# Tongji-MIC-Lab/TDVC

Measured on AMD Instinct MI355X. Metric: 1080p P-frames/sec (encode + reconstruct, lambda=2048 config), higher is better.
Workload: dtype f16; 1 GPU; 1x 1920x1080 (padded 1088x1920) 7-frame synthetic GOP (seed 1234), batch 1, P-frames coded in GOP order; gop=7, batch=1, parallelism=gop-sharded x1, weights=closed-form filler (no checkpoint ships)

## Files before the change

### include/tdvc_hip.h

```cpp
#ifndef TDVC_HIP_H
#define TDVC_HIP_H

#include <stdint.h>

#ifdef __cplusplus
extern "C" {
#endif

#define TDVC_OK 0
#define TDVC_EINVAL (-1)
#define TDVC_ENOSUP (-2)

typedef struct {
  void* p;
  int32_t N, H, W, C;
  int64_t sn;
  int32_t sp;
  int32_t dtype;
} tdvc_fmap;

enum { TDVC_F16 = 0, TDVC_F32 = 1 };
enum { TDVC_ACT_NONE = 0, TDVC_ACT_RELU = 1, TDVC_ACT_LRELU = 2, TDVC_ACT_CLAMP01 = 3, TDVC_ACT_SIGMOID = 4 };
enum { TDVC_GDN_NONE = 0, TDVC_GDN_FWD = 1, TDVC_GDN_INV = 2 };
enum { TDVC_OUT_NHWC = 0,
// ... 18 lines not shown
  int32_t act; float slope;
  int32_t round_before_act;
  tdvc_fmap res;
  tdvc_fmap res2;
  int32_t out_mode;
  int32_t s2d;
  int32_t bcast_T;
  float bcast_slope;
  float* chan_sum;
} tdvc_conv_desc;

int tdvc_abi_version(void);
const char* tdvc_last_error(void);
int tdvc_prepare_device(void);
const char* tdvc_last_conv_kernel(void);


int tdvc_conv_plan(int cin, int kh, int kw, int stride);
int64_t tdvc_conv_packed_bytes(int cout, int cin, int ntaps, int ck);
int tdvc_pack_conv_weights(const float* w_oihw, int cout, int cin_real, int cin, int kh, int kw,
                           int ntaps, const int8_t* tap_dy, const int8_t* tap_dx, int ck, uint16_t* dst);
int tdvc_conv2d(const tdvc_conv_desc* d, void* stream);
int tdvc_conv_chan_sum_rows(const tdvc_conv_desc* d);
const char* tdvc_conv_select(const tdvc_conv_desc* d);
int tdvc_conv2d_f32(const tdvc_conv_desc* d, void* stream);

typedef struct {
  tdvc_fmap x, y;
  const void* w;
  const float* bias;
// ... 222 lines not shown
```

### tdvc_amd/_lib.py

```python
from __future__ import annotations

import ctypes as C
import os

_HERE = os.path.dirname(os.path.abspath(__file__))
LIB_PATH = os.path.join(_HERE, "libtdvc_hip.so")

MAX_TAPS = 49
F16, F32 = 0, 1
ACT_NONE, ACT_RELU, ACT_LRELU, ACT_CLAMP01, ACT_SIGMOID = 0, 1, 2, 3, 4
GDN_NONE, GDN_FWD, GDN_INV = 0, 1, 2
OUT_NHWC, OUT_SHUFFLE2, OUT_NCHW_F32 = 0, 1, 2


class FMapDesc(C.Structure):
    _fields_ = [("p", C.c_void_p), ("N", C.c_int32), ("H", C.c_int32), ("W", C.c_int32), ("C", C.c_int32),
                ("sn", C.c_int64), ("sp", C.c_int32), ("dtype", C.c_int32)]


class ConvDesc(C.Structure):
    _fields_ = [("x", FMapDesc), ("y", FMapDesc), ("w", C.c_void_p), ("bias", C.c_void_p),
                ("cout", C.c_int32), ("ntaps", C.c_int32),
                ("tap_dy", C.c_int8 * MAX_TAPS), ("tap_dx", C.c_int8 * MAX_TAPS),
                ("kh", C.c_int32), ("kw", C.c_int32), ("stride", C.c_int32), ("pad", C.c_int32),
# ... 19 lines not shown
                ("nworkers", C.c_int32), ("cow", C.c_int32), ("ciw", C.c_int32), ("ntaps", C.c_int32), ("cout", C.c_int32), ("cin", C.c_int32),
                ("wblocks", C.c_int32), ("nblocks", C.c_int32)]


_P = C.c_void_p
_FM = C.POINTER(FMapDesc)
_i, _f, _i64 = C.c_int, C.c_float, C.c_int64

SIGNATURES = {
    "tdvc_abi_version": (_i, []),
    "tdvc_conv_chan_sum_rows": (_i, [C.POINTER(ConvDesc)]),
    "tdvc_conv_select": (C.c_char_p, [C.POINTER(ConvDesc)]),
    "tdvc_last_error": (C.c_char_p, []),
    "tdvc_last_conv_kernel": (C.c_char_p, []),
    "tdvc_prepare_device": (_i, []),
    "tdvc_conv_plan": (_i, [_i, _i, _i, _i]),
    "tdvc_conv_packed_bytes": (_i64, [_i, _i, _i, _i]),
    "tdvc_pack_conv_weights": (_i, [_P, _i, _i, _i, _i, _i, _i, _P, _P, _i, _P]),
    "tdvc_conv2d": (_i, [C.POINTER(ConvDesc), _P]),
    "tdvc_conv2d_f32": (_i, [C.POINTER(ConvDesc), _P]),
    "tdvc_pack_conv_weights_indexed": (_i, [_P] * 7 + [_i] * 4 + [_P, _P]),
    "tdvc_pack_conv_weights_indexed_f32": (_i, [_P] * 7 + [_i] * 4 + [_P, _P]),
    "tdvc_pack_job_blocks": (_i64, [_i, _i, _i, _i]),
    "tdvc_pack_conv_weights_batch": (_i, [_P, _P, _i, _i, _P]),
    "tdvc_act_backward": (_i, [_FM, _FM, _FM, _i, _f, _FM, _P]),
    "tdvc_pixel_unshuffle": (_i, [_FM, _FM, _P]),
    "tdvc_bias_grad_work_floats": (_i64, [_i, _i]),
    "tdvc_bias_grad": (_i, [_FM, _i, _P, _f, _P, _P, _i64, _P]),
    "tdvc_copy_cast": (_i, [_FM, _FM, _P]),
    "tdvc_clamp01_backward": (_i, [_FM, _FM, _P]),
# ... 109 lines not shown
```

### tdvc_amd/csrc/common.h

```cpp
#pragma once
#include <hip/hip_runtime.h>
#include <stdint.h>
#include <stdio.h>
#include <string.h>

#include "../../include/tdvc_hip.h"

typedef _Float16 half_t;
typedef _Float16 half8 __attribute__((ext_vector_type(8)));
typedef _Float16 half4 __attribute__((ext_vector_type(4)));
typedef _Float16 half2v __attribute__((ext_vector_type(2)));
typedef float f32x16 __attribute__((ext_vector_type(16)));
typedef float f32x4 __attribute__((ext_vector_type(4)));

void tdvc_set_error(const char* fmt, ...);
int tdvc_scratch_pages(const void** zeros, void** dump);

#define TDVC_CHECK(cond, ...)            \
  do {                                   \
    if (!(cond)) {                       \
      tdvc_set_error(__VA_ARGS__);       \
      return TDVC_EINVAL;                \
    }                                    \
  } while (0)

static inline int tdvc_launch_status(const char* what) {
  hipError_t e = hipGetLastError();
  if (e != hipSuccess) {
    tdvc_set_error("%s: launch failed: %s", what, hipGetErrorString(e));
    return (int)e;
  }
  return TDVC_OK;
}

static inline bool aligned16(const void* p) { return (((uintptr_t)p) & 15) == 0; }
struct TdvcPerDeviceFlag {
  bool done[64] = {};
  bool& flag() {
    int dev = 0;
    if (hipGetDevice(&dev) != hipSuccess || dev < 0 || dev >= 64) dev = 0;
    return done[dev];
// ... 46 lines not shown
```

### tdvc_amd/csrc/conv_c8.hip

```cpp
#include "conv_common.h"

using convk::ConvParams;

namespace {

constexpr int NW_C8 = 4, NTHR_C8 = 256;
constexpr int EW_C8 = 32 * 144;
constexpr int LDS_C8 = 256 + NW_C8 * EW_C8;

__global__ __launch_bounds__(NTHR_C8, 4) void conv_c8_kernel(const ConvParams p, int tiles_x, int total_tiles) {
  extern __shared__ __attribute__((aligned(16))) unsigned char smem[];
  float* bias_s = reinterpret_cast<float*>(smem);
  const int tid = threadIdx.x, lane = tid & 63;
  const int wave = __builtin_amdgcn_readfirstlane(tid >> 6);
  const int hh = lane >> 5, r = lane & 31;
  if (tid < 64) bias_s[tid] = p.bias[tid];
  unsigned char* ew = smem + 256 + wave * EW_C8;

  half8 wa[2][5];
#pragma unroll
  for (int mt = 0; mt < 2; ++mt)
#pragma unroll
    for (int s = 0; s < 5; ++s) wa[mt][s] = *reinterpret_cast<const half8*>(p.w + (((long)mt * 5 + s) * 64 + lane) * 8);

  int tdy[5], tdx[5];
// ... 70 lines not shown
    }
  }
}

}

bool conv_c8_eligible(const tdvc_conv_desc* d, const ConvParams& p, int Ho, int Wo) {
  return convk::taps_dense(d, 3, 3, 1) && d->ck == 8 && d->stride == 1 && d->cout == 64 && d->x.C == 8 && !d->s2d && !d->square_input &&
         (long)Ho * Wo >= convk::LARGE_MAP_PIXELS &&
         convk::conv_is_lean(p) && !p.res.p && !p.res2.p && p.y.C >= 64 && (long)d->x.N * Ho * ((Wo + 31) / 32) < (1L << 30);
}

int launch_conv_c8(const ConvParams& p, int N, hipStream_t st) {
  ConvParams q = p;
  q.slope = convk::conv_simple_slope(p);
  const int tiles_x = (p.Wo + 31) / 32;
  const long total = (long)N * p.Ho * tiles_x;
  int grid = (int)((total + NW_C8 - 1) / NW_C8);
  if (grid > 256 * 4) grid = 256 * 4;
  hipLaunchKernelGGL(conv_c8_kernel, dim3(grid), dim3(NTHR_C8), LDS_C8, st, q, tiles_x, (int)total);
  return tdvc_launch_status("tdvc_conv2d(c8)");
}
```

### tdvc_amd/csrc/conv_common.h

```cpp
#pragma once
#include "common.h"

namespace convk {

struct ConvParams {
  const half_t* x; long x_sn; int x_sp; int H, W, Cin;
  const half_t* w; const float* bias;
  FMap y; int Ho, Wo; int cout;
  FMap aux; FMap res; FMap res2;
  int ntaps, kh, kw, pad;
  int in_stride;
  int nchunks, steps;
  int square, gdn, act; float slope; int round16, out_mode;
  int tiles_x;
  int simple;
  int s2d, Corig;
  int reverse;
  int bcast_T; float bcast_slope;
  float* csum;
  int8_t tap_dy[TDVC_MAX_TAPS], tap_dx[TDVC_MAX_TAPS];
};

enum ConvSwitch { SW_NONE = -1, SW_V2, SW_V3, SW_V5, SW_V7, SW_V9, SW_V10, SW_V11, SW_ROW, SW_C8, SW_N16, SW_GDN128, SW_COUNT };
int conv_on(int id);
long conv_v9_work_limit();

constexpr long LARGE_MAP_PIXELS = 8192;

inline bool taps_dense(const tdvc_conv_desc* d, int kh, int kw, int pad) {
  if (d->ntaps != kh * kw || d->kh != kh || d->kw != kw || d->pad != pad) return false;
  for (int t = 0; t < d->ntaps; ++t)
    if (d->tap_dy[t] != t / kw || d->tap_dx[t] != t % kw) return false;
  return true;
}

// ... 450 lines not shown
```

### tdvc_amd/csrc/conv_pair.hip

```cpp
#include <type_traits>

#include "conv_common.h"

namespace {

constexpr int BI = 2;
constexpr int TRING = 2 * BI;
constexpr int SRING = 2 * BI;
constexpr int T_LAG = 1 + BI;
constexpr int ID_LAG = 2 + BI;
template <int NCB> struct PairGeoBase;
template <> struct PairGeoBase<2> { static constexpr int PIECES = 5, XRING = 16, PF = 8, HD = 4; };
template <> struct PairGeoBase<4> { static constexpr int PIECES = 9, XRING = 10, PF = 4, HD = 2; };
template <int NCB> struct PairGeo : PairGeoBase<NCB> {
  using G = PairGeoBase<NCB>;
  static constexpr int PW = 16 * NCB - 2;
  static constexpr int NPX = PW + 4;
  static constexpr int ROWB = G::PIECES * 1024;
  static constexpr int TROWB = ROWB;
  static constexpr int SROW = 16 * NCB * 128;
  static constexpr int X0 = 0, T0 = G::XRING * ROWB, S0 = T0 + TRING * TROWB;
  static constexpr int LDS = S0 + SRING * SROW;
  static_assert(NPX * 128 <= ROWB, "ring row holds the strip's input pixels");
  static_assert(G::PF - G::XRING < -(BI - 1) - ID_LAG, "input ring: a DMA would land on a row whose identity a conv2 wave BI - 1 steps behind has not read (needs PF + 2 BI + 2 <= XRING)");
// ... 16 lines not shown
#define PAIR_MID_G 1
#endif

struct PairParams {
  const half_t* x; long x_sn; int x_sp;
  half_t* y; long y_sn; int y_sp;
  const half_t* res2; long r2_sn; int r2_sp;
  const half_t* w;
  const float* bias;
  const half_t* zeros;
  half_t* dump;
  int N, H, W;
  int strips, segs, seg_rows, jobs;
  float slope1, slope2;
  int experiment;
};

__device__ __forceinline__ int swz(int q) { return (int)((0x62654210u >> (4 * ((q >> 1) & 7))) & 7u); }

__device__ __forceinline__ void glds16(const half_t* gsrc, unsigned lds_dst) {
  unsigned keep;
  asm volatile("s_mov_b32 %0, m0\n\ts_mov_b32 m0, %2\n\ts_nop 0\n\tglobal_load_lds_dwordx4 %1, off\n\ts_mov_b32 m0, %0"
               : "=&s"(keep) : "v"(gsrc), "s"(lds_dst) : "memory");
}
__device__ __forceinline__ void pair_barrier(bool skip = false) {
  asm volatile("s_waitcnt lgkmcnt(0)" ::: "memory");
  if (!skip) __builtin_amdgcn_s_barrier();
  asm volatile("" ::: "memory");
}
template <int A>
// ... 3 lines not shown
    return __builtin_elementwise_max(v, z);
  } else if constexpr (A == 2) {
    return __builtin_elementwise_max(v, v * sl);
  } else {
    return v;
  }
}

template <int XRING> __device__ __forceinline__ int pair_slot(int kk) {
  if constexpr ((XRING & (XRING - 1)) == 0) return kk & (XRING - 1);
  else return __builtin_amdgcn_readfirstlane(kk) % XRING;
}

template <int NCB, int A1, int A2, bool ADDX, bool RES2, bool STAMP = false>
__global__ __launch_bounds__(NTHR, 1) void conv_pair_kernel(const PairParams p, long long* stamps = nullptr, int stamp_cap = 0) {
  using G = PairGeo<NCB>;
  constexpr int PW = G::PW, ROWB = G::ROWB, TROWB = G::TROWB, SROW = G::SROW, XRING = G::XRING, PF = G::PF, X0 = G::X0, T0 = G::T0, S0 = G::S0;
  constexpr int NF = 6 * NCB;
  constexpr int NIT = NCB / 2;
  long long st_busy = 0, st_vm = 0, st_bar = 0, st_n = 0;
  extern __shared__ __attribute__((aligned(1024))) unsigned char smem[];
  const unsigned lds0 = static_cast<unsigned>(reinterpret_cast<uintptr_t>(smem));
  const int tid = threadIdx.x, lane = tid & 63;
  const int wave = __builtin_amdgcn_readfirstlane(tid >> 6);
  const int grp = wave >> 2, wq = wave & 3;
  const int r16 = lane & 15, kb = lane >> 4;

  half8 wf[18];
#pragma unroll
  for (int f = 0; f < 18; ++f) wf[f] = *reinterpret_cast<const half8*>(p.w + ((((long)(grp * 4 + wq) * 18 + f) * 64 + lane) * 8));
// ... 359 lines not shown
  const int PWsel = 16 * ncb - 2;
  p.strips = (p.W + PWsel - 1) / PWsel;
  const long base = (long)p.N * p.strips;
  int best = 1;
  double best_eff = 0.;
  for (int sg = 1; sg <= 64 && (p.H + sg - 1) / sg >= 16; ++sg) {
    const int sr = (p.H + sg - 1) / sg, nseg = (p.H + sr - 1) / sr;
    const long jobs = base * nseg;
    const double eff = (double)jobs / (double)(((jobs + 255) / 256) * 256) * sr / (sr + 5.0);
    if (eff > best_eff + 1e-9) { best_eff = eff; best = sg; }
  }
  p.seg_rows = (p.H + best - 1) / best;
  p.segs = (p.H + p.seg_rows - 1) / p.seg_rows;
  p.jobs = (int)(base * p.segs);
  const int grid = p.jobs < 256 ? p.jobs : 256;
  auto go = [&](auto kern, int lds) -> int {
    hipError_t err = hipFuncSetAttribute(reinterpret_cast<const void*>(kern), hipFuncAttributeMaxDynamicSharedMemorySize, lds);
    if (err != hipSuccess) { tdvc_set_error("tdvc_conv_pair: hipFuncSetAttribute failed: %s", hipGetErrorString(err)); return (int)err; }
    hipLaunchKernelGGL(kern, dim3(grid), dim3(NTHR), lds, reinterpret_cast<hipStream_t>(stream), p, g_pair_stamps, g_pair_stamp_cap);
    return 0;
  };
  const bool resblock = d->act1 == TDVC_ACT_RELU && d->act2 == TDVC_ACT_NONE;
  const int sel = (resblock ? 4 : 0) + (d->add_input ? 2 : 0) + (d->res2.p ? 1 : 0);
  auto launch = [&](auto ncbc) -> int {
    constexpr int NCB = decltype(ncbc)::value;
    constexpr int lds = PairGeo<NCB>::LDS;
    switch (sel) {
      case 0: return go(&conv_pair_kernel<NCB, 2, 2, false, false>, lds);
      case 1: return go(&conv_pair_kernel<NCB, 2, 2, false, true>, lds);
      case 2: return go(&conv_pair_kernel<NCB, 2, 2, true, false>, lds);
// ... 12 lines not shown
```

### tdvc_amd/csrc/conv_row.hip

```cpp
#include <type_traits>

#include "conv_common.h"

using convk::ConvParams;

namespace {

enum { GEO_C128 = 0, GEO_C64 = 1, GEO_C128W = 2, GEO_S2D64 = 3 };
template <int GID> struct RowGeo;
template <> struct RowGeo<GEO_C128> { static constexpr int NKC = 4, KH = 3, KW = 3, SW = 32, NCG = 8, PIECES = 9, XRING = 8, PF = 6, HD = 4, DMA_POS = 1, CORIG = 128; static constexpr bool S2D = false; };
template <> struct RowGeo<GEO_C64> { static constexpr int NKC = 2, KH = 3, KW = 3, SW = 64, NCG = 4, PIECES = 9, XRING = 8, PF = 6, HD = 4, DMA_POS = 2, CORIG = 64; static constexpr bool S2D = false; };
template <> struct RowGeo<GEO_C128W> { static constexpr int NKC = 4, KH = 3, KW = 3, SW = 64, NCG = 4, PIECES = 17, XRING = 6, PF = 4, HD = 2, DMA_POS = 2, CORIG = 128; static constexpr bool S2D = false; };
template <> struct RowGeo<GEO_S2D64> { static constexpr int NKC = 8, KH = 2, KW = 2, SW = 32, NCG = 8, PIECES = 17, XRING = 6, PF = 4, HD = 2, DMA_POS = 1, CORIG = 64; static constexpr bool S2D = true; };
template <int GID> struct RowDerived : RowGeo<GID> {
  using G = RowGeo<GID>;
  static constexpr int CO = 16 * G::NCG;
  static constexpr int PXB = G::NKC * 64;
  static constexpr int LPP = PXB / 16;
  static constexpr int SLOTS = CO / 8;
  static constexpr int ROWB = G::PIECES * 1024;
  static constexpr int STEPS = (G::KH * G::KW * 4 + 1) / 2;
  static constexpr int NP = G::PIECES / 4 + 1;
  static constexpr int X0 = 0, S0 = G::XRING * ROWB, B0 = S0 + 4 * 8192, LDS = B0 + 512;
  static_assert(G::SW * CO * 2 == 8192, "a staging row is 8 KB = 512 items of 16 bytes");
// ... 14 lines not shown
struct RowParams {
  const half_t* x; long x_sn; int x_sp;
  half_t* y; long y_sn; int y_sp;
  const half_t* res; long r1_sn; int r1_sp;
  const half_t* w;
  const float* bias;
  const half_t* zeros;
  half_t* dump;
  int N, H, W;
  int Win;
  int ncb;
  int cq;
  int strips;
  float slope;
  int reverse;
};

template <int PXB> __device__ __forceinline__ int rw_f(int q) {
  return PXB == 128 ? ((q >> 1) & 7) : ((q & 12) | ((q & 1) << 1) | ((q >> 1) & 1));
}
__device__ __forceinline__ int rw_sigma(int r) { return r < 4 ? 2 * r : (r >= 12 ? 2 * r - 16 : 2 * r - 7); }
__device__ __forceinline__ int rw_g(int q) { return (q >> 1) & 7; }

__device__ __forceinline__ void rw_glds16(const half_t* gsrc, unsigned lds_dst) {
  unsigned keep;
  asm volatile("s_mov_b32 %0, m0\n\ts_mov_b32 m0, %2\n\ts_nop 0\n\tglobal_load_lds_dwordx4 %1, off\n\ts_mov_b32 m0, %0"
               : "=&s"(keep) : "v"(gsrc), "s"(lds_dst) : "memory");
}
template <int XRING> __device__ __forceinline__ int rw_slot(int kk) {
  if constexpr ((XRING & (XRING - 1)) == 0) return kk & (XRING - 1);
// ... 28 lines not shown
      if (n == i) return g;
      ++n;
    }
  return -1;
}
template <int GID> constexpr int rw_first_group_of_row0() {
  for (int i = 0; i < rw_ngroups<GID>(); ++i) {
    const int g = rw_group_at<GID>(i);
    if (rw_frag<GID>(0, g % RowGeo<GID>::KW, g / RowGeo<GID>::KW)) return i;
  }
  return -1;
}

template <int GID, int ACT, int NRES, bool SHUF>
__global__ __launch_bounds__(RW_NTHR, 1) void conv_row_kernel(const RowParams p) {
  using G = RowDerived<GID>;
  constexpr int NKC = G::NKC, KH = G::KH, KW = G::KW, SW = G::SW, CO = G::CO, PXB = G::PXB, XRING = G::XRING, PF = G::PF, NP = G::NP;
  constexpr int NG = rw_ngroups<GID>(), G0 = rw_first_group_of_row0<GID>();
  extern __shared__ __attribute__((aligned(1024))) unsigned char smem[];
  const unsigned lds0 = static_cast<unsigned>(reinterpret_cast<uintptr_t>(smem));
  const int tid = threadIdx.x, lane = tid & 63;
  const int wave = __builtin_amdgcn_readfirstlane(tid >> 6);
  const bool loader = wave < 4;
  const int wq = wave & 3;
  const int cg = wave % G::NCG, cbp = wave / G::NCG;
  const int r16 = lane & 15, kb = lane >> 4;

  const int nwg = (int)gridDim.x, b = (int)blockIdx.x;
  int cbk, pos_slot, nslots;
  if ((nwg & 7) == 0 && ((nwg >> 3) % p.ncb) == 0) {
// ... 292 lines not shown
  q.cq = shuf ? p.cout >> 2 : 0;
  q.slope = convk::conv_simple_slope(p);
  q.reverse = p.reverse;
  q.strips = (q.W + G::SW - 1) / G::SW;
  const long allrows = (long)N * q.strips * q.H;
  int per = 256 / q.ncb;
  if (per < 1) per = 1;
  if (allrows < per) per = (int)allrows;
  const int grid = per * q.ncb;
  if (!p.res.p && p.res2.p) {
    q.res = reinterpret_cast<const half_t*>(p.res2.p); q.r1_sn = p.res2.sn; q.r1_sp = p.res2.sp;
  }
  const bool has1 = q.res != nullptr;
  const int act = q.slope == 1.f ? 0 : (q.slope == 0.f ? 1 : 2);
  const int nres = has1 ? 1 : 0;
  int rc = TDVC_EINVAL;
#define RW_CASE(A, R, S) \
  if (act == A && nres == R && shuf == S) \
    rc = convk::launch_big_lds<&conv_row_kernel<GID, A, R, S>>("tdvc_conv2d(conv_row)", G::LDS, dim3(grid), dim3(RW_NTHR), G::LDS, st, q);
  RW_CASE(0, 0, false) RW_CASE(0, 1, false) RW_CASE(1, 0, false) RW_CASE(1, 1, false) RW_CASE(2, 0, false) RW_CASE(2, 1, false)
  if constexpr (GID == GEO_C128) {
    RW_CASE(0, 0, true) RW_CASE(0, 1, true) RW_CASE(1, 0, true) RW_CASE(1, 1, true) RW_CASE(2, 0, true) RW_CASE(2, 1, true)
  }
#undef RW_CASE
  return rc;
}

int launch_conv_row(int geo, const ConvParams& p, int N, hipStream_t st) {
  switch (geo) {
    case GEO_C128: return launch_conv_row_t<GEO_C128>(p, N, st);
// ... 6 lines not shown
```

### tdvc_amd/csrc/lib.cpp

```cpp
#include <hip/hip_runtime.h>
#include <stdarg.h>
#include <stdio.h>

#include <mutex>

#include "../../include/tdvc_hip.h"

static thread_local char g_err[512] = "";

void tdvc_set_error(const char* fmt, ...) {
  va_list ap;
  va_start(ap, fmt);
  vsnprintf(g_err, sizeof(g_err), fmt, ap);
  va_end(ap);
}

extern "C" int tdvc_abi_version(void) { return 6; }
extern "C" const char* tdvc_last_error(void) { return g_err; }

namespace {
constexpr int kMaxDev = 64;
constexpr size_t kZeroBytes = 4096, kDumpBytes = 16384;
std::mutex g_scratch_mu;
unsigned char* g_scratch[kMaxDev] = {};
}

int tdvc_scratch_pages(const void** zeros, void** dump) {
  int dev = 0;
  hipError_t err = hipGetDevice(&dev);
  if (err != hipSuccess || dev < 0 || dev >= kMaxDev) {
    tdvc_set_error("scratch pages: hipGetDevice failed or device index %d out of range: %s", dev, hipGetErrorString(err));
    return err != hipSuccess ? (int)err : TDVC_EINVAL;
  }
// ... 20 lines not shown
```

### tdvc_amd/csrc/pointwise.hip

```cpp
#include "pointwise_common.h"

namespace {

__global__ void nchw_to_fmap_kernel(const float* src, int C, FMap y) {
  const long npix = (long)y.H * y.W;
  const long i = (long)blockIdx.x * blockDim.x + threadIdx.x;
  if (i >= npix * y.N) return;
  const int n = (int)(i / npix);
  const long pix = i % npix;
  for (int c0 = 0; c0 < y.C; c0 += 8) {
    float v[8];
#pragma unroll
    for (int j = 0; j < 8; ++j) v[j] = (c0 + j < C) ? src[((long)n * C + c0 + j) * npix + pix] : 0.f;
    store8(y, n, pix, c0, v);
  }
}

__global__ void fmap_to_nchw_kernel(FMap x, int C, float* dst) {
  const long npix = (long)x.H * x.W;
  const long i = (long)blockIdx.x * blockDim.x + threadIdx.x;
  if (i >= npix * x.N) return;
  const int n = (int)(i / npix);
  const long pix = i % npix;
  for (int c0 = 0; c0 < C; c0 += 8) {
// ... 366 lines not shown
  const int y0 = (int)sy < x.H - 1 ? (int)sy : x.H - 1, x0 = (int)sx < x.W - 1 ? (int)sx : x.W - 1;
  const int y1 = y0 + (y0 < x.H - 1), x1 = x0 + (x0 < x.W - 1);
  const float ly1 = sy - y0, lx1 = sx - x0, ly0 = 1.f - ly1, lx0 = 1.f - lx1;
  const float* xp = reinterpret_cast<const float*>(x.p) + (long)n * x.sn;
  float* yp = reinterpret_cast<float*>(y.p) + (long)n * y.sn + pix * y.sp;
  for (int c = 0; c < y.C; ++c) {
    const float a = xp[((long)y0 * x.W + x0) * x.sp + c], b = xp[((long)y0 * x.W + x1) * x.sp + c];
    const float cc = xp[((long)y1 * x.W + x0) * x.sp + c], d = xp[((long)y1 * x.W + x1) * x.sp + c];
    float v = ly0 * (lx0 * a + lx1 * b) + ly1 * (lx0 * cc + lx1 * d);
    if (chscale) v *= chscale[c];
    yp[c] = v;
  }
}

constexpr int POOL_ROWS = 8;
__global__ __launch_bounds__(256) void avgpool_k_strip_kernel(FMap x, int scale, float* work, int wp, int nsplit) {
  __shared__ float red[256][9];
  const int chunks = x.C / 8;
  const int lanes = 256 / chunks;
  const int tid = threadIdx.x;
  const int ck = tid % chunks, pl = tid / chunks;
  const int cell = blockIdx.x / nsplit, strip = blockIdx.x - cell * nsplit, n = blockIdx.y;
  const int py = cell / wp, px = cell % wp;
  const int r0 = strip * POOL_ROWS, rows = min(POOL_ROWS, scale - r0);
  float acc[8];
#pragma unroll
  for (int j = 0; j < 8; ++j) acc[j] = 0.f;
  const int area = rows * scale;
  if (pl < lanes) {
    int k = pl;
    for (; k + 3 * lanes < area; k += 4 * lanes) {
      float v[4][8];
// ... 13 lines not shown
#pragma unroll
      for (int j = 0; j < 8; ++j) acc[j] += v[j];
    }
  }
#pragma unroll
  for (int j = 0; j < 8; ++j) red[tid][j] = (pl < lanes) ? acc[j] : 0.f;
  __syncthreads();
  if (tid < x.C) {
    const int cc = tid / 8, j = tid % 8;
    float s = 0.f;
    for (int l = 0; l < lanes; ++l) s += red[l * chunks + cc][j];
    work[(((long)n * gridDim.x) + blockIdx.x) * x.C + tid] = s;
  }
}

__global__ void avgpool_k_final_kernel(const float* work, float* pooled, long total, int C_, int nsplit, float area) {
  const long i = (long)blockIdx.x * blockDim.x + threadIdx.x;
  if (i >= total) return;
  const long cell = i / C_;
  const int c = (int)(i - cell * C_);
  float s = 0.f;
  for (int k = 0; k < nsplit; ++k) s += work[(cell * nsplit + k) * C_ + c];
  pooled[i] = s / area;
}

__device__ __forceinline__ float block_sum(float v, float* sh) {
  const int tid = threadIdx.x;
#pragma unroll
  for (int o = 32; o > 0; o >>= 1) v += __shfl_xor(v, o);
  __syncthreads();
  if ((tid & 63) == 0) sh[tid >> 6] = v;
  __syncthreads();
  return sh[0] + sh[1] + sh[2] + sh[3];
}

__device__ __forceinline__ float patch_elem(const float* pm, int hp, int wp, int C, int pi, int pj, int d) {
  const int c = d / 9, k = d % 9;
  const int yy = 3 * pi - 3 + k / 3, xx = 3 * pj - 3 + k % 3;
// ... 289 lines not shown
  TDVC_CHECK(x && y && fmap_ok32(*x) && fmap_ok32(*y) && y->C <= x->C && y->N == x->N, "tdvc_resize_bilinear: bad arguments");
  const long total = (long)y->N * y->H * y->W;
  hipLaunchKernelGGL(resize_bilinear_kernel, grid1d(total), dim3(EW_BLOCK), 0, ST(stream), to_dev(*x), to_dev(*y), chscale);
  return tdvc_launch_status("tdvc_resize_bilinear");
}

extern "C" int64_t tdvc_avgpool_k_work_floats(int N, int hp, int wp, int C_, int scale) {
  return (int64_t)N * hp * wp * ((scale + POOL_ROWS - 1) / POOL_ROWS) * C_;
}

extern "C" int tdvc_avgpool_k(const tdvc_fmap* x, int scale, float* pooled, int hp, int wp, float* work, int64_t work_floats, void* stream) {
  TDVC_CHECK(x && pooled && work && fmap_ok16(*x) && x->C <= 256 && scale >= 1 && hp == x->H / scale && wp == x->W / scale && hp >= 1 && wp >= 1,
             "tdvc_avgpool_k: bad arguments");
  const int nsplit = (scale + POOL_ROWS - 1) / POOL_ROWS;
  TDVC_CHECK(work_floats >= tdvc_avgpool_k_work_floats(x->N, hp, wp, x->C, scale), "tdvc_avgpool_k: workspace too small (tdvc_avgpool_k_work_floats)");
  hipLaunchKernelGGL(avgpool_k_strip_kernel, dim3(hp * wp * nsplit, x->N), dim3(256), 0, ST(stream), to_dev(*x), scale, work, wp, nsplit);
  const long total = (long)x->N * hp * wp * x->C;
  hipLaunchKernelGGL(avgpool_k_final_kernel, grid1d(total), dim3(256), 0, ST(stream), work, pooled, total, x->C, nsplit, (float)scale * (float)scale);
  return tdvc_launch_status("tdvc_avgpool_k");
}

extern "C" int tdvc_patch_match(const float* pin, const float* pref, int N, int hp, int wp, int C, int32_t* idx, void* stream) {
  TDVC_CHECK(pin && pref && idx && N >= 1 && hp >= 1 && wp >= 1 && C >= 1 && C * 9 * 4 <= 60000, "tdvc_patch_match: bad arguments");
  const int nph = (hp + 3) / 3 + 1, npw = (wp + 3) / 3 + 1;
  hipLaunchKernelGGL(patch_match_kernel, dim3(nph * npw, N), dim3(256), (size_t)C * 9 * 4, ST(stream), pin, pref, hp, wp, C, nph, npw, idx);
  return tdvc_launch_status("tdvc_patch_match");
}

extern "C" int tdvc_match_gather(const tdvc_fmap* fin, const tdvc_fmap* fref, const int32_t* idx, int scale, int hp, int wp,
                                 const tdvc_fmap* cat, void* stream) {
  TDVC_CHECK(fin && fref && idx && cat && fmap_ok16(*fin) && fmap_ok16(*fref) && fmap_ok16(*cat), "tdvc_match_gather: bad fmaps");
  TDVC_CHECK(fin->C == 64 && fref->C == 64 && cat->C == 128 && same_geom(*fin, *fref) && same_geom(*fin, *cat), "tdvc_match_gather: needs C=64 / cat C=128");
  const int ks = 3 * scale;
  const int nbh = (fin->H + ks) / ks + 1, nbw = (fin->W + ks) / ks + 1;
// ... 40 lines not shown
```

### tdvc_amd/model/modules.py

```python
from __future__ import annotations

import torch
import torch.nn as nn

from .. import ops
from ..ops import ACT_LRELU, ACT_NONE, ACT_RELU, FM


class PackCache:

    def _pk(self, key, fn):
        c = self.__dict__.setdefault("_packed", {})
        if key not in c:
            c[key] = fn()
        return c[key]


def _dev(m: nn.Module):
    return next(m.parameters()).device


def pk_conv(owner: PackCache, name: str, conv: nn.Module, **kw) -> ops.PackedConv:
    def build():
        w = conv.weight
# ... 308 lines not shown

class FeatureExtract(nn.Module, PackCache):

    def __init__(self, cin, mid, nblocks):
        super().__init__()
        self.conv_first = nn.Conv2d(cin, mid, 3, 1, 1)
        self.body = res_stack(nblocks, mid)
        self.conv_last = nn.Conv2d(mid, mid, 3, 1, 1)

    def run(self, x: FM, out: FM | None = None) -> FM:
        x1 = ops.conv(x, pk_conv(self, "first", self.conv_first), act=ACT_LRELU, slope=0.01)
        t = run_stack(self.body, x1)
        return ops.conv(t, pk_conv(self, "last", self.conv_last), out=out, res=x1)


class FeatureFix(nn.Module, PackCache):

    def __init__(self):
        super().__init__()
        self.FeatureExtract_input = FeatureExtract(64, 64, 2)
        self.FeatureExtract_ref = FeatureExtract(3, 64, 2)
        self.recon_layer = res_stack(2)
        self.conv_10 = nn.Conv2d(64, 64, 3, 2, 1)
        self.conv_11 = nn.Conv2d(64, 64, 3, 1, 1)
        self.conv_12 = nn.Conv2d(64, 64, 3, 2, 1)
        self.conv_13 = nn.Conv2d(64, 64, 3, 1, 1)
        self.featfusion = nn.Conv2d(128, 64, 3, 1, 1)
        self.featfusion2 = nn.Conv2d(128, 64, 3, 1, 1)
        self.featdown = nn.Conv2d(64, 3, 3, 1, 1)
        self.attn = SELayer(64)

    def run(self, x: FM, iframe8: FM, training: bool, trace=None) -> torch.Tensor:
        B, H, W = x.N, x.H, x.W
        dev = x.t.device
        lr = dict(act=ACT_LRELU, slope=0.1)
        fin = self.FeatureExtract_input.run(x)
        y = FM.empty(B, H, W, 128, device=dev)
        fref = self.FeatureExtract_ref.run(iframe8, out=y.ch(64, 64))
        scale = 8 if training else int(H / 8)
        pin, pref = ops.avgpool_k(fin, scale), ops.avgpool_k(fref, scale)
        idx = ops.patch_match(pin, pref)
        cat = FM.empty(B, H, W, 128, device=dev)
        ops.match_gather(fin, fref, idx, scale, cat)
        ops.conv(cat, pk_conv(self, "ff", self.featfusion), out=y.ch(0, 64), **lr)
        sums = []
        o2 = ops.conv(y, pk_conv(self, "ff2", self.featfusion2), chan_sum=sums)
        o2 = self.attn.run(o2, sums=sums, **lr)
        o = run_stack(self.recon_layer, o2, res2=x)
        rgb = torch.empty((B, 3, H, W), dtype=torch.float32, device=dev)
        ops.conv(o, pk_conv(self, "down", self.featdown), act=ops.ACT_CLAMP01, nchw_out=rgb)
        if trace is not None:
            trace.update(ff_idx=idx, ff_fin=fin, ff_fref=fref)
        return rgb
```

### tdvc_amd/ops.py

```python
from __future__ import annotations

import ctypes as C
from dataclasses import dataclass

import numpy as np
import torch

from . import _lib as L
from . import convpack
from ._lib import (ACT_CLAMP01, ACT_LRELU, ACT_NONE, ACT_RELU, GDN_FWD, GDN_INV, GDN_NONE, OUT_NCHW_F32,
                   OUT_NHWC, OUT_SHUFFLE2)


_raw_stream = torch._C._cuda_getCurrentRawStream
_cur_dev = torch._C._cuda_getDevice
FORCE_STREAM = None
FORCE_KEEP = None


def _stream():
    if FORCE_STREAM is not None:
        return C.c_void_p(FORCE_STREAM)
    return C.c_void_p(_raw_stream(_cur_dev()))


PROFILE = None
TAPE = None
_IN_BACKWARD = False


def _rec(name, *args):
    if TAPE is not None and not _IN_BACKWARD:
        from . import autograd
        getattr(autograd, "record_" + name)(TAPE, *args)


def pad8(c: int) -> int:
    return (c + 7) // 8 * 8


class FM:

    __slots__ = ("t", "off", "N", "C", "H", "W", "sn", "sp", "_d")
# ... 380 lines not shown
        raise L.TdvcHipError("conv: bcast_T is an inference-only fusion (under the tape use conv + bcast_add_act)")
    if PROFILE is not None:
        e0, e1 = torch.cuda.Event(enable_timing=True), torch.cuda.Event(enable_timing=True)
        e0.record()
        L.check(L.lib().tdvc_conv2d(C.byref(d), _stream()), "conv2d")
        e1.record()
        PROFILE.append(dict(kernel=L.lib().tdvc_last_conv_kernel().decode(),
                            shape=f"{pc.kh}x{pc.kw} s{pc.stride} {x.C}->{pc.cout} @{x.H}x{x.W}" + (" f32out" if out_dtype == torch.float32 else "") + (" nchw" if nchw_out is not None else ""),
                            e0=e0, e1=e1,
                            flops=2.0 * x.N * Ho * Wo * pc.cout * x.C * len(pc.taps),
                            flops_real=(x.N * Ho * Wo * pc.flops_per_px) if pc.s2d else 2.0 * x.N * Ho * Wo * pc.cout * pc.cin_real * len(pc.taps),
                            bytes=2.0 * x.N * (x.H * x.W * x.C + Ho * Wo * pc.cout * (4 if pc.shuffle else 1) / (4 if pc.shuffle else 1))))
        _rec("conv", x, rec_pc, None if nchw_out is not None else ret, act, slope, res, res2, gdn, aux, square, nchw_out)
        return ret
    L.check(L.lib().tdvc_conv2d(C.byref(d), _stream()), "conv2d")
    _rec("conv", x, rec_pc, None if nchw_out is not None else ret, act, slope, res, res2, gdn, aux, square, nchw_out)
    return ret


class PackedConvPair:

    def __init__(self, w: torch.Tensor, bias: torch.Tensor):
        self.w, self.bias = w, bias


def pack_conv_pair(w1: torch.Tensor, b1: torch.Tensor | None, w2: torch.Tensor, b2: torch.Tensor | None) -> PackedConvPair:
    for w in (w1, w2):
        if tuple(w.shape) != (64, 64, 3, 3):
            raise L.TdvcHipError(f"pack_conv_pair: weights must be (64, 64, 3, 3), got {tuple(w.shape)}")
    frag = lambda w: w.detach().float().reshape(4, 16, 2, 4, 8, 9).permute(0, 5, 2, 3, 1, 4)
# ... 28 lines not shown
    if TAPE is not None:
        raise L.TdvcHipError("conv_pair: inference only (the intermediate map is not kept for the backward pass)")
    if out is None:
        out = FM.empty(x.N, x.H, x.W, 64, device=x.t.device)
    d = _pair_desc(x, pp, out, act1, slope1, act2, slope2, add_input, res2)
    if PROFILE is not None:
        e0, e1 = torch.cuda.Event(enable_timing=True), torch.cuda.Event(enable_timing=True)
        e0.record()
        L.check(L.lib().tdvc_conv_pair(C.byref(d), _stream()), "conv_pair")
        e1.record()
        fl = 2 * 2.0 * x.N * x.H * x.W * 64 * 64 * 9
        PROFILE.append(dict(kernel="conv_pair", shape=f"2x(3x3 s1 64->64) @{x.H}x{x.W}", e0=e0, e1=e1, flops=fl, flops_real=fl,
                            bytes=2.0 * x.N * x.H * x.W * 128))
        return out
    L.check(L.lib().tdvc_conv_pair(C.byref(d), _stream()), "conv_pair")
    return out


def act_backward(g: FM, y: FM, act, slope=0.0, res: FM | None = None, out: FM | None = None) -> FM:
    out = g if out is None else out
    dg, dy, do = g.desc(), y.desc(), out.desc()
    dr = res.desc() if res is not None else None
    L.check(L.lib().tdvc_act_backward(C.byref(dg), C.byref(dy), C.byref(dr) if dr is not None else None, act, slope, C.byref(do), _stream()),
            "act_backward")
    return out


def pixel_unshuffle(y: FM, out: FM | None = None) -> FM:
    if out is None:
        out = FM.empty(y.N, y.H // 2, y.W // 2, 4 * y.C, dtype=y.t.dtype, device=y.t.device)
# ... 382 lines not shown
def resize_bilinear(x: FM, H: int, W: int, chscale: torch.Tensor | None = None) -> FM:
    out = FM.empty(x.N, H, W, x.C, dtype=torch.float32, device=x.t.device)
    dx, dy = x.desc(), out.desc()
    L.check(L.lib().tdvc_resize_bilinear(C.byref(dx), C.byref(dy), chscale.data_ptr() if chscale is not None else None,
                                         _stream()), "resize_bilinear")
    _rec("resize_bilinear", x, out, chscale)
    return out


def resize_bilinear_backward(dy: FM, dx: FM, chscale: torch.Tensor | None = None) -> None:
    d1, d2 = dy.desc(), dx.desc()
    L.check(L.lib().tdvc_resize_bilinear_backward(C.byref(d1), C.byref(d2), chscale.data_ptr() if chscale is not None else None, _stream()),
            "resize_bilinear_backward")


def avgpool_k(x: FM, scale: int) -> torch.Tensor:
    hp, wp = x.H // scale, x.W // scale
    pooled = torch.empty((x.N, hp, wp, x.C), dtype=torch.float32, device=x.t.device)
    nwork = L.lib().tdvc_avgpool_k_work_floats(x.N, hp, wp, x.C, scale)
    work = torch.empty((nwork,), dtype=torch.float32, device=x.t.device)
    dx = x.desc()
    L.check(L.lib().tdvc_avgpool_k(C.byref(dx), scale, pooled.data_ptr(), hp, wp, work.data_ptr(), nwork, _stream()), "avgpool_k")
    return pooled


def patch_match(pin: torch.Tensor, pref: torch.Tensor) -> torch.Tensor:
    N, hp, wp, Cc = pin.shape
    Lp = ((hp + 3) // 3 + 1) * ((wp + 3) // 3 + 1)
    idx = torch.empty((N, Lp), dtype=torch.int32, device=pin.device)
    L.check(L.lib().tdvc_patch_match(pin.data_ptr(), pref.data_ptr(), N, hp, wp, Cc, idx.data_ptr(), _stream()),
            "patch_match")
    return idx


def match_gather(fin: FM, fref: FM, idx: torch.Tensor, scale: int, cat: FM):
    df, dr, dc = fin.desc(), fref.desc(), cat.desc()
    L.check(L.lib().tdvc_match_gather(C.byref(df), C.byref(dr), idx.data_ptr(), scale, fin.H // scale, fin.W // scale,
# ... 280 lines not shown
```

### tdvc_amd/train.py

```python
from __future__ import annotations

import gc
from collections.abc import Mapping

import torch
import torch.distributed as dist

from . import autograd, ops
from .synth import split_optim_params


def refresh_packed(model: torch.nn.Module) -> None:
    pcs = []
    mods = model.__dict__.get("_mods_list")
    if mods is None:
        mods = model.__dict__["_mods_list"] = list(model.modules())
    from .model.coder import GDN, gdn_refresh_batched
    pcs += gdn_refresh_batched([m for m in mods if isinstance(m, GDN)])
    for m in mods:
        m.__dict__.pop("_ar_cache", None)
        if isinstance(m, GDN):
            continue
        if hasattr(m, "refresh_packed"):
            m.refresh_packed()
            continue
        pk = m.__dict__.get("_packed", {})
        pcs += [pc for pc in pk.values() if isinstance(pc, ops.PackedConv)]
        for key in [k for k, v in pk.items() if isinstance(v, ops.PackedConvPair)]:
            del pk[key]
    batch = model.__dict__.get("_pack_batch")
    if batch is None or batch.forms != ops.FORMS_CREATED or [id(pc) for pc in batch.roots] != [id(pc) for pc in pcs]:
        batch = ops.PackBatch(pcs)
        batch.roots = pcs
        model.__dict__["_pack_batch"] = batch
    batch.run()


class GradBuckets:

    def __init__(self, params, bucket_bytes: int = 16 << 20):
        self.params = [p for p in params if p.requires_grad]
# ... 291 lines not shown
```

Measured before the change: 47.60 frames/s.

## Skip redundant I-frame feature extraction via device-side predicated kernels

FeatureFix now caches the reference I-frame's extracted features and pooled descriptors in persistent buffers. Each call first runs a GPU compare kernel against a cached copy of the I-frame and writes a change flag. The conv, conv-pair, conv-row and avgpool kernels of the reference chain are then launched with a device predicate that makes them exit immediately when the flag is zero. This removes the repeated full-resolution reference feature extraction for P-frames that share one I-frame, with no host sync. The cost is an extra compare/copy pass, persistent buffers, still-issued launches, and a fallback path if any kernel in the chain cannot be predicated.

```diff
diff --git a/include/tdvc_hip.h b/include/tdvc_hip.h
--- a/include/tdvc_hip.h
+++ b/include/tdvc_hip.h
@@ -56,6 +56,10 @@
 const char* tdvc_last_error(void);
 int tdvc_prepare_device(void);
 const char* tdvc_last_conv_kernel(void);
+
+int tdvc_set_predicate(const int* flag);
+int tdvc_last_launch_predicated(void);
+int tdvc_frame_changed(const tdvc_fmap* cur, tdvc_fmap* cache, int* flag, void* stream);
 
 
 int tdvc_conv_plan(int cin, int kh, int kw, int stride);
diff --git a/tdvc_amd/_lib.py b/tdvc_amd/_lib.py
--- a/tdvc_amd/_lib.py
+++ b/tdvc_amd/_lib.py
@@ -57,6 +57,9 @@
     "tdvc_last_error": (C.c_char_p, []),
     "tdvc_last_conv_kernel": (C.c_char_p, []),
     "tdvc_prepare_device": (_i, []),
+    "tdvc_set_predicate": (_i, [_P]),
+    "tdvc_last_launch_predicated": (_i, []),
+    "tdvc_frame_changed": (_i, [_FM, _FM, _P, _P]),
     "tdvc_conv_plan": (_i, [_i, _i, _i, _i]),
     "tdvc_conv_packed_bytes": (_i64, [_i, _i, _i, _i]),
     "tdvc_pack_conv_weights": (_i, [_P, _i, _i, _i, _i, _i, _i, _P, _P, _i, _P]),
diff --git a/tdvc_amd/csrc/common.h b/tdvc_amd/csrc/common.h
--- a/tdvc_amd/csrc/common.h
+++ b/tdvc_amd/csrc/common.h
@@ -16,6 +16,13 @@
 void tdvc_set_error(const char* fmt, ...);
 int tdvc_scratch_pages(const void** zeros, void** dump);
 
+const int* tdvc_launch_predicate();
+void tdvc_note_launch();
+#define TDVC_PREDICATE_RETURN(pred)                       \
+  do {                                                    \
+    if ((pred) != nullptr && *(pred) == 0) return;        \
+  } while (0)
+
 #define TDVC_CHECK(cond, ...)            \
   do {                                   \
     if (!(cond)) {                       \
@@ -25,6 +32,7 @@
   } while (0)
 
 static inline int tdvc_launch_status(const char* what) {
+  tdvc_note_launch();
   hipError_t e = hipGetLastError();
   if (e != hipSuccess) {
     tdvc_set_error("%s: launch failed: %s", what, hipGetErrorString(e));
diff --git a/tdvc_amd/csrc/conv_c8.hip b/tdvc_amd/csrc/conv_c8.hip
--- a/tdvc_amd/csrc/conv_c8.hip
+++ b/tdvc_amd/csrc/conv_c8.hip
@@ -9,6 +9,7 @@
 constexpr int LDS_C8 = 256 + NW_C8 * EW_C8;
 
 __global__ __launch_bounds__(NTHR_C8, 4) void conv_c8_kernel(const ConvParams p, int tiles_x, int total_tiles) {
+  TDVC_PREDICATE_RETURN(p.pred);
   extern __shared__ __attribute__((aligned(16))) unsigned char smem[];
   float* bias_s = reinterpret_cast<float*>(smem);
   const int tid = threadIdx.x, lane = tid & 63;
@@ -109,6 +110,7 @@
 int launch_conv_c8(const ConvParams& p, int N, hipStream_t st) {
   ConvParams q = p;
   q.slope = convk::conv_simple_slope(p);
+  q.pred = tdvc_launch_predicate();
   const int tiles_x = (p.Wo + 31) / 32;
   const long total = (long)N * p.Ho * tiles_x;
   int grid = (int)((total + NW_C8 - 1) / NW_C8);
diff --git a/tdvc_amd/csrc/conv_common.h b/tdvc_amd/csrc/conv_common.h
--- a/tdvc_amd/csrc/conv_common.h
+++ b/tdvc_amd/csrc/conv_common.h
@@ -19,6 +19,7 @@
   int bcast_T; float bcast_slope;
   float* csum;
   int8_t tap_dy[TDVC_MAX_TAPS], tap_dx[TDVC_MAX_TAPS];
+  const int* pred;
 };
 
 enum ConvSwitch { SW_NONE = -1, SW_V2, SW_V3, SW_V5, SW_V7, SW_V9, SW_V10, SW_V11, SW_ROW, SW_C8, SW_N16, SW_GDN128, SW_COUNT };
diff --git a/tdvc_amd/csrc/conv_pair.hip b/tdvc_amd/csrc/conv_pair.hip
--- a/tdvc_amd/csrc/conv_pair.hip
+++ b/tdvc_amd/csrc/conv_pair.hip
@@ -54,6 +54,7 @@
   int strips, segs, seg_rows, jobs;
   float slope1, slope2;
   int experiment;
+  const int* pred;
 };
 
 __device__ __forceinline__ int swz(int q) { return (int)((0x62654210u >> (4 * ((q >> 1) & 7))) & 7u); }
@@ -87,6 +88,7 @@
 
 template <int NCB, int A1, int A2, bool ADDX, bool RES2, bool STAMP = false>
 __global__ __launch_bounds__(NTHR, 1) void conv_pair_kernel(const PairParams p, long long* stamps = nullptr, int stamp_cap = 0) {
+  TDVC_PREDICATE_RETURN(p.pred);
   using G = PairGeo<NCB>;
   constexpr int PW = G::PW, ROWB = G::ROWB, TROWB = G::TROWB, SROW = G::SROW, XRING = G::XRING, PF = G::PF, X0 = G::X0, T0 = G::T0, S0 = G::S0;
   constexpr int NF = 6 * NCB;
@@ -476,6 +478,7 @@
   p.segs = (p.H + p.seg_rows - 1) / p.seg_rows;
   p.jobs = (int)(base * p.segs);
   const int grid = p.jobs < 256 ? p.jobs : 256;
+  p.pred = tdvc_launch_predicate();
   auto go = [&](auto kern, int lds) -> int {
     hipError_t err = hipFuncSetAttribute(reinterpret_cast<const void*>(kern), hipFuncAttributeMaxDynamicSharedMemorySize, lds);
     if (err != hipSuccess) { tdvc_set_error("tdvc_conv_pair: hipFuncSetAttribute failed: %s", hipGetErrorString(err)); return (int)err; }
diff --git a/tdvc_amd/csrc/conv_row.hip b/tdvc_amd/csrc/conv_row.hip
--- a/tdvc_amd/csrc/conv_row.hip
+++ b/tdvc_amd/csrc/conv_row.hip
@@ -52,6 +52,7 @@
   int strips;
   float slope;
   int reverse;
+  const int* pred;
 };
 
 template <int PXB> __device__ __forceinline__ int rw_f(int q) {
@@ -110,6 +111,7 @@
 
 template <int GID, int ACT, int NRES, bool SHUF>
 __global__ __launch_bounds__(RW_NTHR, 1) void conv_row_kernel(const RowParams p) {
+  TDVC_PREDICATE_RETURN(p.pred);
   using G = RowDerived<GID>;
   constexpr int NKC = G::NKC, KH = G::KH, KW = G::KW, SW = G::SW, CO = G::CO, PXB = G::PXB, XRING = G::XRING, PF = G::PF, NP = G::NP;
   constexpr int NG = rw_ngroups<GID>(), G0 = rw_first_group_of_row0<GID>();
@@ -432,6 +434,7 @@
   const bool has1 = q.res != nullptr;
   const int act = q.slope == 1.f ? 0 : (q.slope == 0.f ? 1 : 2);
   const int nres = has1 ? 1 : 0;
+  q.pred = tdvc_launch_predicate();
   int rc = TDVC_EINVAL;
 #define RW_CASE(A, R, S) \
   if (act == A && nres == R && shuf == S) \
diff --git a/tdvc_amd/csrc/lib.cpp b/tdvc_amd/csrc/lib.cpp
--- a/tdvc_amd/csrc/lib.cpp
+++ b/tdvc_amd/csrc/lib.cpp
@@ -15,8 +15,26 @@
   va_end(ap);
 }
 
-extern "C" int tdvc_abi_version(void) { return 6; }
+extern "C" int tdvc_abi_version(void) { return 7; }
 extern "C" const char* tdvc_last_error(void) { return g_err; }
+
+static thread_local const int* g_pred = nullptr;
+static thread_local int g_pred_taken = 0, g_pred_last = 0;
+
+extern "C" int tdvc_set_predicate(const int* flag) {
+  if (reinterpret_cast<uintptr_t>(flag) & 3) { tdvc_set_error("tdvc_set_predicate: flag must be 4-byte aligned"); return TDVC_EINVAL; }
+  g_pred = flag;
+  return TDVC_OK;
+}
+extern "C" int tdvc_last_launch_predicated(void) { return g_pred_last; }
+const int* tdvc_launch_predicate() {
+  g_pred_taken = g_pred != nullptr;
+  return g_pred;
+}
+void tdvc_note_launch() {
+  g_pred_last = g_pred_taken;
+  g_pred_taken = 0;
+}
 
 namespace {
 constexpr int kMaxDev = 64;
diff --git a/tdvc_amd/csrc/pointwise.hip b/tdvc_amd/csrc/pointwise.hip
--- a/tdvc_amd/csrc/pointwise.hip
+++ b/tdvc_amd/csrc/pointwise.hip
@@ -404,8 +404,9 @@
 }
 
 constexpr int POOL_ROWS = 8;
-__global__ __launch_bounds__(256) void avgpool_k_strip_kernel(FMap x, int scale, float* work, int wp, int nsplit) {
+__global__ __launch_bounds__(256) void avgpool_k_strip_kernel(FMap x, int scale, float* work, int wp, int nsplit, const int* pred) {
   __shared__ float red[256][9];
+  TDVC_PREDICATE_RETURN(pred);
   const int chunks = x.C / 8;
   const int lanes = 256 / chunks;
   const int tid = threadIdx.x;
@@ -449,7 +450,8 @@
   }
 }
 
-__global__ void avgpool_k_final_kernel(const float* work, float* pooled, long total, int C_, int nsplit, float area) {
+__global__ void avgpool_k_final_kernel(const float* work, float* pooled, long total, int C_, int nsplit, float area, const int* pred) {
+  TDVC_PREDICATE_RETURN(pred);
   const long i = (long)blockIdx.x * blockDim.x + threadIdx.x;
   if (i >= total) return;
   const long cell = i / C_;
@@ -457,6 +459,28 @@
   float s = 0.f;
   for (int k = 0; k < nsplit; ++k) s += work[(cell * nsplit + k) * C_ + c];
   pooled[i] = s / area;
+}
+
+typedef unsigned int u32x4 __attribute__((ext_vector_type(4)));
+__device__ __forceinline__ u32x4* frame_word(const FMap& f, long i) {
+  const int c8 = f.C / 8;
+  const long per_img = (long)f.H * f.W * c8;
+  const long n = i / per_img, rem = i - n * per_img;
+  const long pix = rem / c8;
+  const int ck = (int)(rem - pix * c8);
+  return reinterpret_cast<u32x4*>(reinterpret_cast<half_t*>(f.p) + n * f.sn + pix * f.sp + ck * 8);
+}
+__global__ __launch_bounds__(EW_BLOCK) void frame_compare_kernel(FMap cur, FMap cache, long words, int* flag) {
+  const long i = (long)blockIdx.x * blockDim.x + threadIdx.x;
+  if (i >= words) return;
+  const u32x4 a = *frame_word(cur, i), b = *frame_word(cache, i);
+  if (((a[0] ^ b[0]) | (a[1] ^ b[1]) | (a[2] ^ b[2]) | (a[3] ^ b[3])) != 0u) flag[0] = 1;
+}
+__global__ __launch_bounds__(EW_BLOCK) void frame_refresh_kernel(FMap cur, FMap cache, long words, const int* flag) {
+  if (flag[0] == 0) return;
+  const long i = (long)blockIdx.x * blockDim.x + threadIdx.x;
+  if (i >= words) return;
+  *frame_word(cache, i) = *frame_word(cur, i);
 }
 
 __device__ __forceinline__ float block_sum(float v, float* sh) {
@@ -776,10 +800,22 @@
              "tdvc_avgpool_k: bad arguments");
   const int nsplit = (scale + POOL_ROWS - 1) / POOL_ROWS;
   TDVC_CHECK(work_floats >= tdvc_avgpool_k_work_floats(x->N, hp, wp, x->C, scale), "tdvc_avgpool_k: workspace too small (tdvc_avgpool_k_work_floats)");
-  hipLaunchKernelGGL(avgpool_k_strip_kernel, dim3(hp * wp * nsplit, x->N), dim3(256), 0, ST(stream), to_dev(*x), scale, work, wp, nsplit);
+  const int* pred = tdvc_launch_predicate();
+  hipLaunchKernelGGL(avgpool_k_strip_kernel, dim3(hp * wp * nsplit, x->N), dim3(256), 0, ST(stream), to_dev(*x), scale, work, wp, nsplit, pred);
   const long total = (long)x->N * hp * wp * x->C;
-  hipLaunchKernelGGL(avgpool_k_final_kernel, grid1d(total), dim3(256), 0, ST(stream), work, pooled, total, x->C, nsplit, (float)scale * (float)scale);
+  hipLaunchKernelGGL(avgpool_k_final_kernel, grid1d(total), dim3(256), 0, ST(stream), work, pooled, total, x->C, nsplit, (float)scale * (float)scale, pred);
   return tdvc_launch_status("tdvc_avgpool_k");
+}
+
+extern "C" int tdvc_frame_changed(const tdvc_fmap* cur, tdvc_fmap* cache, int* flag, void* stream) {
+  TDVC_CHECK(cur && cache && flag && fmap_ok16(*cur) && fmap_ok16(*cache) && same_geom(*cur, *cache) && cur->C == cache->C &&
+             (reinterpret_cast<uintptr_t>(flag) & 3) == 0, "tdvc_frame_changed: fp16 maps of one geometry and a 4-byte aligned flag");
+  const hipError_t err = hipMemsetAsync(flag, 0, sizeof(int), ST(stream));
+  if (err != hipSuccess) { tdvc_set_error("tdvc_frame_changed: hipMemsetAsync failed: %s", hipGetErrorString(err)); return (int)err; }
+  const long words = (long)cur->N * cur->H * cur->W * (cur->C / 8);
+  hipLaunchKernelGGL(frame_compare_kernel, grid1d(words), dim3(EW_BLOCK), 0, ST(stream), to_dev(*cur), to_dev(*cache), words, flag);
+  hipLaunchKernelGGL(frame_refresh_kernel, grid1d(words), dim3(EW_BLOCK), 0, ST(stream), to_dev(*cur), to_dev(*cache), words, flag);
+  return tdvc_launch_status("tdvc_frame_changed");
 }
 
 extern "C" int tdvc_patch_match(const float* pin, const float* pref, int N, int hp, int wp, int C, int32_t* idx, void* stream) {
diff --git a/tdvc_amd/model/modules.py b/tdvc_amd/model/modules.py
--- a/tdvc_amd/model/modules.py
+++ b/tdvc_amd/model/modules.py
@@ -346,6 +346,18 @@
         return ops.conv(t, pk_conv(self, "last", self.conv_last), out=out, res=x1)
 
 
+FEATUREFIX_REUSE = True
+
+
+class IFrameReuse:
+
+    __slots__ = ("key", "y", "iframe", "pref", "flag", "usable", "log")
+
+    def __init__(self, key):
+        self.key, self.usable, self.log = key, None, []
+        self.y = self.iframe = self.pref = self.flag = None
+
+
 class FeatureFix(nn.Module, PackCache):
 
     def __init__(self):
@@ -367,10 +379,15 @@
         dev = x.t.device
         lr = dict(act=ACT_LRELU, slope=0.1)
         fin = self.FeatureExtract_input.run(x)
-        y = FM.empty(B, H, W, 128, device=dev)
-        fref = self.FeatureExtract_ref.run(iframe8, out=y.ch(64, 64))
         scale = 8 if training else int(H / 8)
-        pin, pref = ops.avgpool_k(fin, scale), ops.avgpool_k(fref, scale)
+        if FEATUREFIX_REUSE and not training and ops.TAPE is None and ops.PROFILE is None and trace is None and not iframe8.f32:
+            y, pref = self._iframe_features(iframe8, scale)
+            fref = y.ch(64, 64)
+        else:
+            y = FM.empty(B, H, W, 128, device=dev)
+            fref = self.FeatureExtract_ref.run(iframe8, out=y.ch(64, 64))
+            pref = ops.avgpool_k(fref, scale)
+        pin = ops.avgpool_k(fin, scale)
         idx = ops.patch_match(pin, pref)
         cat = FM.empty(B, H, W, 128, device=dev)
         ops.match_gather(fin, fref, idx, scale, cat)
@@ -384,3 +401,47 @@
         if trace is not None:
             trace.update(ff_idx=idx, ff_fin=fin, ff_fref=fref)
         return rgb
+
+    def reuse_state(self) -> IFrameReuse | None:
+        return self.__dict__.get("_packed", {}).get("iframe_reuse")
+
+    def _iframe_features(self, iframe8: FM, scale: int):
+        B, H, W = iframe8.N, iframe8.H, iframe8.W
+        dev = iframe8.t.device
+        key = (dev.index, ops._stream().value, B, H, W, scale)
+        cache = self.__dict__.setdefault("_packed", {})
+        st = cache.get("iframe_reuse")
+        if st is None or st.key != key:
+            st = cache["iframe_reuse"] = IFrameReuse(key)
+
+        def chain(y, pref):
+            fref = self.FeatureExtract_ref.run(iframe8, out=y.ch(64, 64))
+            ops.avgpool_k(fref, scale, out=pref)
+
+        def fresh():
+            return (FM.empty(B, H, W, 128, device=dev),
+                    torch.empty((B, H // scale, W // scale, 64), dtype=torch.float32, device=dev))
+
+        if st.usable is False:
+            y, pref = fresh()
+            chain(y, pref)
+            return y, pref
+        if st.usable is None:
+            st.y, st.pref = fresh()
+            st.iframe = FM.empty(B, H, W, iframe8.C, device=dev)
+            st.flag = torch.ones(1, dtype=torch.int32, device=dev)
+            ops.copy_cast(iframe8, st.iframe)
+        else:
+            ops.frame_changed(iframe8, st.iframe, st.flag)
+        with ops.predicate(st.flag) as log:
+            chain(st.y, st.pref)
+        st.log = list(log)
+        y, pref = st.y, st.pref
+        if not all(log):
+            if st.usable is not None:
+                chain(y, pref)
+            st.usable = False
+            st.y = st.iframe = st.pref = st.flag = None
+        else:
+            st.usable = True
+        return y, pref
diff --git a/tdvc_amd/ops.py b/tdvc_amd/ops.py
--- a/tdvc_amd/ops.py
+++ b/tdvc_amd/ops.py
@@ -27,6 +27,40 @@
 PROFILE = None
 TAPE = None
 _IN_BACKWARD = False
+
+
+_PRED_LOG = None
+
+
+class predicate:
+
+    def __init__(self, flag: torch.Tensor):
+        assert flag.dtype == torch.int32 and flag.is_cuda and flag.numel() >= 1
+        self.flag = flag
+
+    def __enter__(self):
+        global _PRED_LOG
+        if _PRED_LOG is not None:
+            raise L.TdvcHipError("ops.predicate does not nest")
+        L.check(L.lib().tdvc_set_predicate(self.flag.data_ptr()), "set_predicate")
+        _PRED_LOG = []
+        return _PRED_LOG
+
+    def __exit__(self, *exc):
+        global _PRED_LOG
+        _PRED_LOG = None
+        L.lib().tdvc_set_predicate(None)
+        return False
+
+
+def _log_predicated(kernels=1):
+    if _PRED_LOG is not None:
+        _PRED_LOG.extend([bool(L.lib().tdvc_last_launch_predicated())] * kernels)
+
+
+def frame_changed(cur: FM, cache: FM, flag: torch.Tensor) -> None:
+    dc, dk = cur.desc(), cache.desc()
+    L.check(L.lib().tdvc_frame_changed(C.byref(dc), C.byref(dk), flag.data_ptr(), _stream()), "frame_changed")
 
 
 def _rec(name, *args):
@@ -437,6 +471,7 @@
         _rec("conv", x, rec_pc, None if nchw_out is not None else ret, act, slope, res, res2, gdn, aux, square, nchw_out)
         return ret
     L.check(L.lib().tdvc_conv2d(C.byref(d), _stream()), "conv2d")
+    _log_predicated()
     _rec("conv", x, rec_pc, None if nchw_out is not None else ret, act, slope, res, res2, gdn, aux, square, nchw_out)
     return ret
 
@@ -495,6 +530,7 @@
                             bytes=2.0 * x.N * x.H * x.W * 128))
         return out
     L.check(L.lib().tdvc_conv_pair(C.byref(d), _stream()), "conv_pair")
+    _log_predicated()
     return out
 
 
@@ -907,13 +943,15 @@
             "resize_bilinear_backward")
 
 
-def avgpool_k(x: FM, scale: int) -> torch.Tensor:
+def avgpool_k(x: FM, scale: int, out: torch.Tensor | None = None) -> torch.Tensor:
     hp, wp = x.H // scale, x.W // scale
-    pooled = torch.empty((x.N, hp, wp, x.C), dtype=torch.float32, device=x.t.device)
+    pooled = torch.empty((x.N, hp, wp, x.C), dtype=torch.float32, device=x.t.device) if out is None else out
+    assert pooled.shape == (x.N, hp, wp, x.C) and pooled.dtype == torch.float32 and pooled.is_contiguous()
     nwork = L.lib().tdvc_avgpool_k_work_floats(x.N, hp, wp, x.C, scale)
     work = torch.empty((nwork,), dtype=torch.float32, device=x.t.device)
     dx = x.desc()
     L.check(L.lib().tdvc_avgpool_k(C.byref(dx), scale, pooled.data_ptr(), hp, wp, work.data_ptr(), nwork, _stream()), "avgpool_k")
+    _log_predicated(2)
     return pooled
 
 
diff --git a/tdvc_amd/train.py b/tdvc_amd/train.py
--- a/tdvc_amd/train.py
+++ b/tdvc_amd/train.py
@@ -25,6 +25,7 @@
             m.refresh_packed()
             continue
         pk = m.__dict__.get("_packed", {})
+        pk.pop("iframe_reuse", None)
         pcs += [pc for pc in pk.values() if isinstance(pc, ops.PackedConv)]
         for key in [k for k, v in pk.items() if isinstance(v, ops.PackedConvPair)]:
             del pk[key]
```

Result: faster. 49.37 frames/s (median of 6 runs) (+3.7%).
